# bayesian-object-tracking/dbot_ros

Hardware: AMD Instinct MI355X
Metric: particle-likelihoods/sec @640x480 (higher is better)
Workload: dtype f64; 1 GPU; C1: 2000 particles/GPU x loglikes(update=true), 640x480 synthetic depth frame, mesh m1 (5120 triangles), parents=permutation, 30-frame moving-object sequence, likelihood precision f64, window planes, inputs resident in HBM; particles_per_gpu=2000, triangles=5120

## Files before the change

dbot_ros_amd/csrc/rbsensor_capi.hip:

```cpp
#include "rbsensor_kernels.hip"
#include "rbsensor_tracker.hip"
#include "rbsensor_peers.hip"
#include "rbs_mesh.h"

#include "../../include/rbsensor_mi355x.h"

#include <dlfcn.h>
#include <unistd.h>
#if defined(__x86_64__)
#include <immintrin.h>
#endif

#include <cmath>
#include <cstdarg>
#include <cstddef>
#include <cstdio>
#include <cstdlib>
#include <cstring>
#include <algorithm>
#include <array>
#include <map>
#include <new>
#include <string>
#include <utility>
// ... 19 lines not shown
    double* d_soup = nullptr;
    float* d_frame = nullptr;
    double* d_aux = nullptr;
    double* d_aux_slot[2] = {nullptr, nullptr};
    float* d_pbg = nullptr;
    float* d_occ[2] = {nullptr, nullptr};
    int cur = 0;
    int pending_frames = 0;
    double* d_poses = nullptr;
    int* d_indices = nullptr;
    int* d_rects[2] = {nullptr, nullptr};
    rbs::Groups* d_groups[2] = {nullptr, nullptr};
    rbs::Strips* d_strips[2] = {nullptr, nullptr};
    int tracker_split_max = RBS_TRACKER_SPLIT_MAX_DEFAULT;
    bool copy_walk = false;
    int* d_parents[2] = {nullptr, nullptr};
    int4* d_win[2] = {nullptr, nullptr};
    int4* d_win_used = nullptr;
    int slab_px = 0;
    size_t plane_stride = 0;
    int4* d_reg[2] = {nullptr, nullptr};
    int* d_err = nullptr;
    int* h_err = nullptr;
    bool slab_auto = false;
    bool slab_probed = false;
    int* d_bbox = nullptr;
    bool windowed = true;
    bool many_clusters = false;
    unsigned char* d_wide_flags = nullptr;
    unsigned long long* d_area = nullptr;
    unsigned long long* h_area = nullptr;
    hipEvent_t ev_area = nullptr;
    bool area_pending = false;
    int area_n = 0;
    bool wide = false;
    double area_frac = 0.0;
    double mid_enter = 0.15;
    bool balance = true;
    int balance_blocks = 0;
    long balance_seen = 0;
    double wide_enter = 0.50, wide_leave = 0.35;
    int cu_count = 256;
    int smalln_target = 768;
    int rect_align = 4;
    int win_chunks = 8;
    int win_chunks_single = 2;
    int upload_chunks = 2;
    bool quiet = false;
    bool async_outstanding = false;
    float background = 0.f;
    int2* d_item_range = nullptr;
    int* d_item_particle = nullptr;
    int* d_ctr = nullptr;
    bool stp = false, stp_allowed = true;
    float* d_bgp[2] = {nullptr, nullptr};
    double stp_enter = 0.10;
    int stp_every = 32;
    long stp_last_rebase = -1000000;
    long stp_rebases = 0;
    long stp_block_until = 0;
    struct StpNow { int rebase = -1; bool entering = false; } stp_now;
    bool stp_leave_pending = false;
    int stp_request = -1;
    bool ipc_exported = false;
    int4* d_bgp_box = nullptr;
    bool split = false;
    unsigned* d_depth = nullptr;
    size_t depth_items = 0;
    int depth_blocks = 0, eval_blocks = 0;
    int* d_done = nullptr;
    double* d_partial = nullptr;
    unsigned long long* d_phase = nullptr;
    size_t partial_cap = 0;
    float* d_cluster_sphere = nullptr;
    float* d_cluster_cone = nullptr;
    double* d_cluster_vtx = nullptr;
    int* d_cluster_nv = nullptr;
    unsigned* d_tri_local = nullptr;
    float* d_vtx = nullptr;
    float* d_tri_plane = nullptr;
    int precision = RBS_PRECISION_F64;
    bool one_body_kernel = true;
    bool fused_copy = true;
    bool exact = false;
    int age_max = 0;
    double* d_ptab = nullptr;
    std::vector<double> ptab;
    long update_clock = 0;
    float* d_tmp_plane = nullptr;
    float* d_render = nullptr;
    unsigned char* h_in = nullptr;
    double* h_out = nullptr;
    unsigned char* d_in = nullptr;
    unsigned char* h_in_dev = nullptr;
    double* h_out_dev = nullptr;
    size_t in_idx_off = 0;
    hipEvent_t ev_out = nullptr;
    float* h_frames[2] = {nullptr, nullptr};
    float* h_frames_dev[2] = {nullptr, nullptr};
    size_t frame_pull_bytes = 128 * 1024;
    hipEvent_t ev_frame[2] = {nullptr, nullptr};
    hipStream_t up_stream = nullptr;
    float* d_fin[2] = {nullptr, nullptr};
    hipEvent_t ev_used[2] = {nullptr, nullptr};
    hipEvent_t ev_reader = nullptr;
    struct NextFrame {
        enum Kind { NONE, BORROWED_F64, BORROWED_F32, DEVICE, AHEAD } kind = NONE;
        const void* src = nullptr;
        hipStream_t stream = nullptr;
        int slot = -1;
        bool borrowed() const { return kind == BORROWED_F64 || kind == BORROWED_F32; }
    };
    struct FrameState {
        int cur = -1;
        int stage = 0;
        bool acquired = false;
        NextFrame next;
    } fr;
    hipStream_t stream = nullptr;
    hipStream_t copy_stream = nullptr;
    hipEvent_t ev_fork = nullptr;
    int copy_blocks = 1 << 30;
    int raster_blocks = 768;
    int copy_rows = 2;
    int copy_tpb = 64;
    const char* tile_override = nullptr;
    static constexpr int kRing = 256;
    hipEvent_t ev_start[kRing] = {}, ev_stop[kRing] = {}, ev_copy_start[kRing] = {}, ev_join[kRing] = {};
    hipEvent_t ev_raster_start[kRing] = {}, ev_raster_stop[kRing] = {}, ev_copy_stop[kRing] = {};
    bool ring_update[kRing] = {};
    int timing_every = 8;
    long timed_calls = 0;
    long calls = 0;
    int join_pending = -1;
    std::string err;
    bool poisoned = false;
    std::string poison_msg;
    int fault_shard = -1;
    long fault_call = -1, group_calls = 0;
    std::vector<rbs_handle*> shards;
    rbs_handle* group = nullptr;
    int shard_index = 0;
    int shard_cap = 0;
    hipEvent_t ev_done = nullptr;
    struct Rccl* rccl = nullptr;
    int peer_world = 0, peer_rank = 0;
    const float* peer_occ[rbs::kMaxDevices][2] = {};
    const int4* peer_win[rbs::kMaxDevices][2] = {};
    const int4* peer_reg[rbs::kMaxDevices][2] = {};
    void* peer_mapped[rbs::kMaxDevices][6] = {};
    void* d_peer_scratch = nullptr;
    size_t peer_scratch_bytes = 0;
    const float* snap_occ[rbs::kMaxDevices] = {};
    const int4* snap_win[rbs::kMaxDevices] = {};
    const int4* snap_reg[rbs::kMaxDevices] = {};
    rbs_config cfg{};
    std::vector<double> cfg_vertices;
    std::vector<int32_t> cfg_vertex_counts, cfg_triangles, cfg_triangle_counts;
    int occ_slots = 0;
};

struct Rccl {
    void* lib = nullptr;
    typedef void* comm_t;
    int (*CommInitAll)(comm_t*, int, const int*) = nullptr;
    int (*CommDestroy)(comm_t) = nullptr;
// ... 651 lines not shown
        const size_t bytes = sizeof(unsigned) * (size_t)rbs::kDepthTilePx * want;
        bool fits = bytes <= kDepthBudget;
        if (fits && want > h->depth_items) {
            size_t free_b = 0, total_b = 0;
            if (hipMemGetInfo(&free_b, &total_b) == hipSuccess) {
                const size_t mine = sizeof(unsigned) * (size_t)rbs::kDepthTilePx * h->depth_items;
                fits = bytes <= (free_b + mine) / 2;
            } else {
                (void)hipGetLastError();
            }
        }
        if (want > h->depth_items && fits) {
            RBS_HIP(h, hipStreamSynchronize(s));
            (void)hipFree(h->d_depth);
            h->d_depth = nullptr;
            h->depth_items = 0;
            if (hipMalloc(&h->d_depth, bytes) == hipSuccess) {
                h->depth_items = want;
            } else {
                (void)hipGetLastError();
                h->d_depth = nullptr;
                fits = false;
            }
        }
        if (want > h->depth_items && !fits) {
            split = false;
            if (have_borrowed) {
                if (int32_t rc = stage_borrowed(h)) return rc;
                P.frame = obs_frame(h);
                P.aux = obs_aux(h);
            }
        }
    }
    if (split) {
        P.depth = h->d_depth;
        P.depth_items = (int)std::min<size_t>(h->depth_items, 0x7fffffff);
        P.ctrb_this = h->d_ctr + 4 + (int)(h->calls & 1);
        P.ctrb_next = h->d_ctr + 4 + (int)((h->calls + 1) & 1);
    }
    int* const d_rects = h->d_rects[h->calls & 1];
    P.rects = d_rects;
    P.groups = h->d_groups[h->calls & 1];
    P.strips = update && h->windowed && !h->copy_walk ? h->d_strips[h->calls & 1] : nullptr;
    P.parents = h->d_parents[h->calls & 1];
    P.item_range = h->d_item_range;
    P.item_particle = h->d_item_particle;
    P.ctr_this = h->d_ctr + 2 * (int)(h->calls & 1);
    P.ctr_next = h->d_ctr + 2 * (int)((h->calls + 1) & 1);
    P.done = h->d_done;
    P.partial = h->d_partial;
#ifdef RBS_PHASE_TIMING
    if (!h->d_phase) { RBS_HIP(h, hipMalloc(&h->d_phase, 256)); RBS_HIP(h, hipMemset(h->d_phase, 0, 256)); }
    P.phase = h->d_phase;
#endif
    if (timed) RBS_HIP(h, hipEventRecord(h->ev_start[tslot], s));
    const dim3 block(rbs::kBlock);
    const dim3 pgrid((unsigned)((n + rbs::kPrepPerBlock - 1) / rbs::kPrepPerBlock));
    if (h->windowed && h->join_pending >= 0) {
        RBS_HIP(h, hipStreamWaitEvent(s, h->ev_join[h->join_pending], 0));
        h->join_pending = -1;
    }
    const float* rb_occ = P.occ_src; const int4* rb_win = P.win_src; const int4* rb_reg = h->slab_px ? P.reg_src : (const int4*)nullptr;
    int rb_local = rebase;
    if (rebase >= 0 && P.n_dev > 1) {
        const int owner = rebase / P.shard_cap;
        rb_local = rebase - owner * P.shard_cap;
        rb_occ = P.occ_src_dev[owner]; rb_win = P.win_src_dev[owner]; rb_reg = h->slab_px ? P.reg_src_dev[owner] : (const int4*)nullptr;
    }
    if (P.bgp_src) P.rebase_box = rebase >= 0 ? rb_win + rb_local : rebase == -2 ? h->d_bgp_box : nullptr;
    if (P.bgp_src && update)
        if (int32_t rc = launch_bgp_step(h, P, rb_occ, rb_win, rb_reg, rebase >= 0 ? rb_local : rebase, s)) return rc;
    bool sample_area = false;
    if (h->windowed && update) {
        sample_area = timed && !h->area_pending;
        if (sample_area) RBS_HIP(h, hipMemsetAsync(h->d_area, 0, sizeof(unsigned long long), s));
    }
    P.area_sum = sample_area ? h->d_area : nullptr;
    const bool wide = h->windowed && update && h->wide;
    const bool mid = h->windowed && update && !wide && h->area_frac > h->mid_enter;
    const bool fused = h->fused_copy && update && h->windowed && !wide && !mid && !split && !h->exact && !h->slab_px && !P.bgp_src &&
                       !P.groups && h->n_bodies == 1 && !h->many_clusters && !h->group && h->peer_world <= 1 && !h->ipc_exported &&
                       (h->precision == RBS_PRECISION_F32 || h->one_body_kernel);
    if (timed && fused) h->ring_update[tslot] = false;
    if (const float* df = take_device_frame(h, s)) {
        constexpr int ptb = 64 * rbs::kPrepPerBlock;
        const int aux_blocks = (h->d_aux || df != h->d_frame) ? (h->npx + ptb - 1) / ptb : 0;
        hipLaunchKernelGGL(rbs::rbs_frame_prep_kernel, dim3((unsigned)(aux_blocks + (n + rbs::kPrepPerBlock - 1) / rbs::kPrepPerBlock)), dim3(ptb), 0, s, P,
                           d_rects, update ? 1 : 0, df, h->d_aux, h->d_pbg, df == h->d_frame ? (float*)nullptr : h->d_frame, aux_blocks);
    } else {
        if (int32_t rc = flush_device_frame(h, s)) return rc;
        if (host_deltas) hipLaunchKernelGGL(rbs::rbs_prep_deltas_kernel, pgrid, dim3(64 * rbs::kPrepPerBlock), 0, s, P, d_rects, update ? 1 : 0);
        else hipLaunchKernelGGL(rbs::rbs_prep_kernel, pgrid, dim3(64 * rbs::kPrepPerBlock), 0, s, P, d_rects, update ? 1 : 0);
    }
    RBS_HIP(h, hipGetLastError());
    if (sample_area) {
        RBS_HIP(h, hipMemcpyAsync(h->h_area, h->d_area, sizeof(unsigned long long), hipMemcpyDeviceToHost, s));
        RBS_HIP(h, hipEventRecord(h->ev_area, s));
        h->area_pending = true;
        h->area_n = (n + 7) / 8;
    }
    if (update && !fused) {
        RBS_HIP(h, hipEventRecord(h->ev_fork, s));
        if (!(h->windowed && !wide)) RBS_HIP(h, hipStreamWaitEvent(h->copy_stream, h->ev_fork, 0));
    }
    if (h->join_pending >= 0) {
        RBS_HIP(h, hipStreamWaitEvent(s, h->ev_join[h->join_pending], 0));
        h->join_pending = -1;
    }
    if (h->balance && h->windowed && update && !wide && !mid && !fused && h->timed_calls > h->balance_seen && h->raster_blocks == 3 * h->cu_count) {
        const int last = (int)((h->timed_calls - 1) % rbs_handle::kRing);
        if (h->ring_update[last] && hipEventQuery(h->ev_raster_stop[last]) == hipSuccess && hipEventQuery(h->ev_copy_stop[last]) == hipSuccess) {
            float r_ms = 0.f, c_ms = 0.f;
            if (hipEventElapsedTime(&r_ms, h->ev_raster_start[last], h->ev_raster_stop[last]) == hipSuccess &&
                hipEventElapsedTime(&c_ms, h->ev_copy_start[last], h->ev_copy_stop[last]) == hipSuccess && r_ms > 0.f) {
                const int step = std::max(1, h->cu_count / 8), lo = 5 * h->cu_count / 2;
                int cur = h->balance_blocks ? h->balance_blocks : h->raster_blocks;
                if (c_ms > 1.04f * r_ms) cur = std::max(lo, cur - step);
                else if (c_ms < 0.92f * r_ms) cur = std::min(h->raster_blocks, cur + step);
                h->balance_blocks = cur;
            } else {
                (void)hipGetLastError();
            }
            h->balance_seen = h->timed_calls;
        }
    }
    const int full_grid = h->balance && h->balance_blocks && h->windowed && update && !fused ? h->balance_blocks : h->raster_blocks;
    const dim3 rgrid((unsigned)(wide || mid ? std::min(h->raster_blocks, 2 * h->cu_count) : full_grid));
    if (!split) if (int32_t rc = wait_for_upload(h, s)) return rc;
    bool window_copy_launched = false;
    auto launch_window_copy = [&]() -> int32_t {
        RBS_HIP(h, hipStreamWaitEvent(h->copy_stream, h->ev_fork, 0));
        if (timed) RBS_HIP(h, hipEventRecord(h->ev_copy_start[tslot], h->copy_stream));
        const int ny = std::min(n, 32768);
        const int strips = !RBS_COPY_STRIPS ? 0 : !P.groups ? 1 : (P.strips ? 2 : 0);
        const dim3 wg((unsigned)(strips == 1 ? h->win_chunks_single : h->win_chunks), (unsigned)ny, (unsigned)((n + ny - 1) / ny));
#define RBS_X3(S, B, E)                                                                                                             \
        do {                                                                                                                        \
            if (strips == 2) hipLaunchKernelGGL((rbs::rbs_copy_window_kernel<S, 2, B, E>), wg, dim3(64), 0, h->copy_stream, P);      \
            else if (strips == 1) hipLaunchKernelGGL((rbs::rbs_copy_window_kernel<S, 1, B, E>), wg, dim3(64), 0, h->copy_stream, P); \
            else hipLaunchKernelGGL((rbs::rbs_copy_window_kernel<S, 0, B, E>), wg, dim3(64), 0, h->copy_stream, P);                  \
        } while (0)
        switch ((h->exact ? 4 : 0) | (h->slab_px ? 2 : 0) | (P.bgp_src ? 1 : 0)) {
            case 0: RBS_X3(false, false, false); break;  case 1: RBS_X3(false, true, false); break;
            case 2: RBS_X3(true, false, false); break;   case 3: RBS_X3(true, true, false); break;
            case 4: RBS_X3(false, false, true); break;   case 5: RBS_X3(false, true, true); break;
            case 6: RBS_X3(true, false, true); break;    default: RBS_X3(true, true, true); break;
        }
#undef RBS_X3
        RBS_HIP(h, hipGetLastError());
        if (timed) RBS_HIP(h, hipEventRecord(h->ev_copy_stop[tslot], h->copy_stream));
        RBS_HIP(h, hipEventRecord(h->ev_join[slot], h->copy_stream));
        window_copy_launched = true;
        return RBS_OK;
    };
    if (timed) RBS_HIP(h, hipEventRecord(h->ev_raster_start[tslot], s));
    if (split) {
        const bool two = wide || mid;
        const dim3 dgrid((unsigned)(two ? std::min(h->depth_blocks, 2 * h->cu_count) : h->depth_blocks));
        const dim3 egrid((unsigned)(two ? std::min(h->eval_blocks, 3 * h->cu_count) : h->eval_blocks));
        const size_t dsm = rbs::smem_bytes_depth(P.tile_px, h->many_clusters), esm = rbs::smem_bytes(0, true, false, h->exact);
        if (h->many_clusters) hipLaunchKernelGGL((rbs::rbs_depth_kernel<true>), dgrid, block, dsm, s, P);
        else hipLaunchKernelGGL((rbs::rbs_depth_kernel<false>), dgrid, block, dsm, s, P);
        RBS_HIP(h, hipGetLastError());
        static const bool copy_first = [] { const char* e = std::getenv("RBS_SPLIT_COPY_FIRST"); return e ? std::atoi(e) != 0 : true; }();
        if (copy_first && have_borrowed && update && h->windowed && !wide)
            if (int32_t rc = launch_window_copy()) return rc;
// ... 461 lines not shown
    switch (cfg->likelihood_precision) {
        case RBS_PRECISION_DEFAULT:
            h->precision = RBS_PRECISION_LIBRARY_DEFAULT;
            if (const char* m = std::getenv("RBS_PRECISION")) {
                if (!std::strcmp(m, "f64")) h->precision = RBS_PRECISION_F64;
                else if (!std::strcmp(m, "f32")) h->precision = RBS_PRECISION_F32;
            }
            break;
        case RBS_PRECISION_F64: case RBS_PRECISION_F32: h->precision = cfg->likelihood_precision; break;
        default: return fail(h, RBS_ERR_INVALID_ARGUMENT, fmt("likelihood_precision %d", cfg->likelihood_precision));
    }
    if (cfg->state_layout < RBS_STATE_DEFAULT || cfg->state_layout > RBS_STATE_DENSE)
        return fail(h, RBS_ERR_INVALID_ARGUMENT, fmt("state_layout %d", cfg->state_layout));
    if (cfg->state_slab_px < RBS_SLAB_WHOLE_PLANES)
        return fail(h, RBS_ERR_INVALID_ARGUMENT, fmt("state_slab_px %d", cfg->state_slab_px));
    if (cfg->occlusion_mode < RBS_OCC_DEFAULT || cfg->occlusion_mode > RBS_OCC_REFERENCE)
        return fail(h, RBS_ERR_INVALID_ARGUMENT, fmt("occlusion_mode %d", cfg->occlusion_mode));

    DevParams& B = h->base;
    B.rows = h->rows; B.cols = h->cols; B.npx = h->npx;
    B.n_bodies = h->n_bodies;
    B.fx = K[0]; B.fy = K[4]; B.cx = K[2]; B.cy = K[5];
    B.tw = std::max(cfg->tail_weight, RBS_TAIL_WEIGHT_FLOOR); B.ms = cfg->model_sigma; B.sf = cfg->sigma_factor;
    B.lambda = -std::log(0.5) / rbs::kHalfLifeDepth;
    B.cv0 = (1.0 - B.tw) / std::sqrt(M_PI);
    B.bands = copy_bands_for(h->rows, h->cols);
    B.band_rows = (h->rows + B.bands - 1) / B.bands;

    rbs::PreparedMesh mesh;
    {
        const rbs::MeshInput in = {cfg->n_objects, cfg->vertices, cfg->vertex_counts, cfg->triangles, cfg->triangle_counts};
        const bool allow_cull = !(std::getenv("RBS_NO_CULL") && std::atoi(std::getenv("RBS_NO_CULL")));
        std::string why;
        if (const int rc = rbs::prepare_mesh(in, allow_cull, &mesh, &why)) return fail(h, rc, why);
        std::copy(std::begin(mesh.tri_begin), std::end(mesh.tri_begin), B.tri_begin);
        std::copy(std::begin(mesh.tri_end), std::end(mesh.tri_end), B.tri_end);
        std::copy(std::begin(mesh.vtx_begin), std::end(mesh.vtx_begin), B.vtx_begin);
        for (int b = 0; b < h->n_bodies; ++b) {
            B.body_cull[b] = mesh.body_cull[b];
            std::copy(mesh.sphere[b], mesh.sphere[b] + 4, B.sphere[b]);
        }
        B.n_tri = (int)mesh.n_alloc;
    }
    {
        size_t nv = 0, nt = 0;
        for (int b = 0; b < cfg->n_objects; ++b) { nv += (size_t)cfg->vertex_counts[b]; nt += (size_t)cfg->triangle_counts[b]; }
        h->cfg = *cfg;
        h->cfg_vertices.assign(cfg->vertices, cfg->vertices + 3 * nv);
        h->cfg_vertex_counts.assign(cfg->vertex_counts, cfg->vertex_counts + cfg->n_objects);
        h->cfg_triangles.assign(cfg->triangles, cfg->triangles + 3 * nt);
        h->cfg_triangle_counts.assign(cfg->triangle_counts, cfg->triangle_counts + cfg->n_objects);
        h->cfg.vertices = h->cfg_vertices.data();
        h->cfg.vertex_counts = h->cfg_vertex_counts.data();
        h->cfg.triangles = h->cfg_triangles.data();
        h->cfg.triangle_counts = h->cfg_triangle_counts.data();
        h->cfg.n_devices = 0;
        h->cfg.device_ids = nullptr;
    }
    h->many_clusters |= mesh.max_clusters > 64 * (rbs::kBlock / 64);
    if (const char* e = std::getenv("RBS_SHARED_CULL")) h->many_clusters = std::atoi(e) != 0;

    const size_t plane = (size_t)h->npx * sizeof(float);
    RBS_HIP(h, hipStreamCreateWithFlags(&h->stream, hipStreamNonBlocking));
    RBS_HIP(h, hipStreamCreateWithFlags(&h->copy_stream, hipStreamNonBlocking));
    RBS_HIP(h, hipEventCreateWithFlags(&h->ev_fork, hipEventDisableTiming));
    for (int i = 0; i < rbs_handle::kRing; ++i) {
        RBS_HIP(h, hipEventCreate(&h->ev_start[i]));
        RBS_HIP(h, hipEventCreate(&h->ev_stop[i]));
        RBS_HIP(h, hipEventCreate(&h->ev_copy_start[i]));
        RBS_HIP(h, hipEventCreate(&h->ev_join[i]));
        RBS_HIP(h, hipEventCreate(&h->ev_raster_start[i]));
        RBS_HIP(h, hipEventCreate(&h->ev_raster_stop[i]));
        RBS_HIP(h, hipEventCreate(&h->ev_copy_stop[i]));
    }
    {
        hipDeviceProp_t prop;
        RBS_HIP(h, hipGetDeviceProperties(&prop, h->device));
        h->cu_count = std::max(1, prop.multiProcessorCount);
        h->raster_blocks = 3 * h->cu_count;
        if (const char* m = std::getenv("RBS_RASTER_BLOCKS")) h->raster_blocks = std::max(1, std::atoi(m));
        if (const char* m = std::getenv("RBS_SHARED_TRAIL")) h->stp_allowed = std::atoi(m) != 0;
        if (const char* m = std::getenv("RBS_ONE_BODY")) h->one_body_kernel = std::atoi(m) != 0;
        if (const char* m = std::getenv("RBS_FUSED_COPY")) h->fused_copy = std::atoi(m) != 0;
        if (const char* m = std::getenv("RBS_TRACKER_SPLIT_MAX")) h->tracker_split_max = std::atoi(m);
        if (const char* m = std::getenv("RBS_STP_ENTER")) h->stp_enter = std::atof(m);
        if (const char* m = std::getenv("RBS_STP_EVERY")) h->stp_every = std::max(1, std::atoi(m));
        h->split = RBS_SPLIT_DEFAULT != 0;
        if (const char* m = std::getenv("RBS_SPLIT")) h->split = std::atoi(m) != 0;
        h->depth_blocks = RBS_DEPTH_MINWAVES * h->cu_count;
        h->eval_blocks = RBS_EVAL_MINWAVES * h->cu_count;
        if (const char* m = std::getenv("RBS_DEPTH_BLOCKS")) h->depth_blocks = std::max(1, std::atoi(m));
        if (const char* m = std::getenv("RBS_EVAL_BLOCKS")) h->eval_blocks = std::max(1, std::atoi(m));
        h->tile_override = std::getenv("RBS_TILE");
        if (const char* m = std::getenv("RBS_COPY_ROWS")) h->copy_rows = std::atoi(m);
        if (const char* m = std::getenv("RBS_COPY_TPB")) h->copy_tpb = std::max(64, std::atoi(m) / 64 * 64);
        if (cfg->state_layout == RBS_STATE_DENSE) h->windowed = false;
        else if (cfg->state_layout == RBS_STATE_DEFAULT)
            if (const char* m = std::getenv("RBS_STATE")) h->windowed = std::strcmp(m, "dense") != 0;
        h->smalln_target = 2 * std::max(1, prop.multiProcessorCount);
        if (const char* m = std::getenv("RBS_SMALLN_TARGET")) h->smalln_target = std::max(1, std::atoi(m));
        if (const char* m = std::getenv("RBS_MID_ENTER")) h->mid_enter = std::atof(m);
        if (const char* m = std::getenv("RBS_BALANCE")) h->balance = std::atoi(m) != 0;
        if (const char* m = std::getenv("RBS_WIDE_ENTER")) { h->wide_enter = std::atof(m); h->wide_leave = h->wide_enter * 0.67; }
        if (const char* m = std::getenv("RBS_RECT_ALIGN")) h->rect_align = std::atoi(m) >= 16 ? 16 : (std::atoi(m) >= 8 ? 8 : 4);
        if (const char* m = std::getenv("RBS_TIMING_EVERY")) h->timing_every = std::max(1, std::atoi(m));
        if (const char* m = std::getenv("RBS_WIN_CHUNKS")) h->win_chunks = h->win_chunks_single = std::min(1024, std::max(1, std::atoi(m)));
        if (const char* m = std::getenv("RBS_UPLOAD_CHUNKS")) h->upload_chunks = std::min(16, std::max(1, std::atoi(m)));
        if (h->cols & 3) h->windowed = false;
        h->base.rect_align = h->windowed ? h->rect_align : rbs::kRectAlign;
        if (!h->windowed && !std::getenv("RBS_RASTER_BLOCKS")) h->raster_blocks = 2 * std::max(1, prop.multiProcessorCount);
    }
    if (int32_t rc = upload(h, &h->d_soup, mesh.soup)) return rc;
    B.soup = h->d_soup;
    RBS_HIP(h, hipMalloc(&h->d_frame, plane));
    if (h->precision == RBS_PRECISION_F64) {
        RBS_HIP(h, hipMalloc(&h->d_aux, sizeof(double) * rbs::AUX_PLANES * (size_t)h->npx));
        RBS_HIP(h, hipMalloc(&h->d_aux_slot[0], sizeof(double) * rbs::AUX_PLANES * (size_t)h->npx));
        RBS_HIP(h, hipMalloc(&h->d_aux_slot[1], sizeof(double) * rbs::AUX_PLANES * (size_t)h->npx));
        RBS_HIP(h, hipMalloc(&h->d_pbg, plane));
    }
    RBS_HIP(h, hipMalloc(&h->d_render, plane));
    {
        int mode = cfg->occlusion_mode;
        const bool ages_fit = std::exp((65534.0 * h->delta_time) * std::log(h->p_oo - h->p_ov)) <= kExactTau;
        const bool can = h->precision == RBS_PRECISION_F64 && h->windowed && ages_fit;
        if (mode == RBS_OCC_REFERENCE && h->precision == RBS_PRECISION_F64 && h->windowed && !ages_fit)
            return fail(h, RBS_ERR_UNSUPPORTED, fmt("occlusion_mode REFERENCE keeps a 16-bit age per pixel: with p_occluded_occluded - p_occluded_visible = %.6g and "
                                                    "delta_time = %.6g a value has not decayed to 2^-40 of itself after 65 534 frames", h->p_oo - h->p_ov, h->delta_time));
        if (mode == RBS_OCC_DEFAULT) {
            mode = RBS_OCC_LIBRARY_DEFAULT;
            if (const char* m = std::getenv("RBS_OCC")) mode = !std::strcmp(m, "reference") ? RBS_OCC_REFERENCE : !std::strcmp(m, "device") ? RBS_OCC_DEVICE_RULE : mode;
            if (mode == RBS_OCC_REFERENCE && !can) mode = RBS_OCC_DEVICE_RULE;
        } else if (mode == RBS_OCC_REFERENCE && !can) {
            return fail(h, RBS_ERR_UNSUPPORTED, "occlusion_mode REFERENCE needs the binary64 likelihood (likelihood_precision F64) and the windowed "
                                                "state layout (cols a multiple of 4)");
        }
        h->exact = mode == RBS_OCC_REFERENCE;
    }
    if (h->exact) {
        const double cc = h->p_oo - h->p_ov, lc = std::log(cc);
        int K = 0;
        while (K < 65534 && std::exp(((double)K * h->delta_time) * lc) > kExactTau) ++K;
        h->age_max = K;
        h->ptab.resize(2 * (size_t)(K + 1));
        for (int a = 0; a <= K; ++a) {
            const double dt = (double)a * h->delta_time;
            const double pow_c = std::exp(dt * lc);
            h->ptab[2 * a] = pow_c;
            h->ptab[2 * a + 1] = (1.0 - h->p_oo) * (pow_c - 1.0) / (cc - 1.0);
        }
        RBS_HIP(h, hipMalloc(&h->d_ptab, sizeof(double) * h->ptab.size()));
        RBS_HIP(h, hipMemcpy(h->d_ptab, h->ptab.data(), sizeof(double) * h->ptab.size(), hipMemcpyHostToDevice));
        RBS_HIP(h, hipMalloc(&h->d_tmp_plane, plane));
    }
    h->slab_px = 0;
    if (h->windowed && cfg->state_slab_px > 0 && cfg->state_slab_px < h->npx)
        h->slab_px = std::max(1024, (cfg->state_slab_px + 3) & ~3);
    else if (h->windowed && cfg->state_slab_px == 0 && h->max_particles > 8192 && (h->cols & 3) == 0 && h->npx / 8 >= 4096) {
        h->slab_px = (h->npx / 8 + 3) & ~3;
        h->slab_auto = true;
    }
    if (h->slab_px >= h->npx) h->slab_px = 0;
    h->plane_stride = h->slab_px ? (size_t)h->slab_px : (size_t)h->npx;
    if (h->exact) h->plane_stride = exact_stride(h->plane_stride);
    const size_t occ_slots = h->occ_slots > 0 ? (size_t)h->occ_slots : (size_t)h->max_particles;
    RBS_HIP(h, hipMalloc(&h->d_occ[0], occ_alloc_bytes(sizeof(float) * h->plane_stride * occ_slots)));
// ... 2204 lines not shown
```

dbot_ros_amd/csrc/rbsensor_kernels.hip:

```cpp
#pragma once
#include <hip/hip_runtime.h>
#include <math.h>
#include <stdint.h>

#include "rbs_math.h"

namespace rbs {

#ifndef RBS_TILE_PX
#define RBS_TILE_PX 11008
#endif
#ifndef RBS_COPY_UNROLL
#define RBS_COPY_UNROLL 8
#endif
#ifndef RBS_NT
#define RBS_NT 1
#endif
#ifndef RBS_BIG_THRESH
#define RBS_BIG_THRESH 96
#endif
#ifndef RBS_EDGE_FILTER
#define RBS_EDGE_FILTER 0
#endif
#ifndef RBS_PIN_EDGES
#define RBS_PIN_EDGES 1
#endif
#ifndef RBS_SHARE_VERTICES
#define RBS_SHARE_VERTICES 1
#endif

#ifndef RBS_BLOCK
#define RBS_BLOCK 256
#endif
constexpr int kBlock = RBS_BLOCK;
constexpr int kTilePx = RBS_TILE_PX;
constexpr int kTilePxBig = 16384;
#ifndef RBS_MATH_LDS
#define RBS_MATH_LDS 1
#endif
constexpr int kMathTabDoubles = RBS_MATH_LDS ? rbsm::kErfcIntervals * rbsm::kErfcCoefs + rbsm::kLogIntervals * 2 : 0;
constexpr int kMathTabPx = (kMathTabDoubles * 8 + 63) / 64 * 16;
constexpr int kTilePxF64 = kTilePx - kMathTabPx, kTilePxBigF64 = kTilePxBig - kMathTabPx;
#ifndef RBS_BIG_CAP
#define RBS_BIG_CAP 256
#endif
constexpr int kBigCap = RBS_BIG_CAP;
constexpr int kBigThresh = RBS_BIG_THRESH;
constexpr int kCopyUnroll = RBS_COPY_UNROLL;
#ifndef RBS_SCAN_UNROLL
#define RBS_SCAN_UNROLL 2
#endif
#ifndef RBS_SCAN_UNROLL_F64
#define RBS_SCAN_UNROLL_F64 2
#endif
constexpr int kQPlanes_ = 4;
constexpr int kEvalQueue = 128;
constexpr int kTq = kQPlanes_ * kEvalQueue;
#ifndef RBS_RASTER_VGPRS
#define RBS_RASTER_VGPRS 80
#endif
#ifndef RBS_PRETEST_CLUSTERS
#define RBS_PRETEST_CLUSTERS 4
#endif
constexpr int kPre = RBS_PRETEST_CLUSTERS;
static_assert(kPre * 64 + 63 <= kTq && (kTq & (kTq - 1)) == 0, "the triangle ring must hold a step's survivors");
constexpr int kCullSteps = 28;
constexpr int kQPlanes = kQPlanes_;
constexpr int kRectAlign = 16;
constexpr float kSnapTau = 0x1p-18f;
typedef float floatx4 __attribute__((ext_vector_type(4)));
constexpr unsigned kInfBits = 0x7f800000u;
constexpr int kMaxBodies = 16;
constexpr int kMaxDevices = 8;
constexpr double kMaxDepth = 6.0;
constexpr double kHalfLifeDepth = 1.0;

constexpr int kMaxGroups = 4;
struct Groups {
    int n, pad0, pad1, pad2;
    int4 rect[kMaxGroups];
    int first[kMaxGroups];
    unsigned mask[kMaxGroups];
};

constexpr int kMaxStrips = (2 * kMaxGroups + 1) * (kMaxGroups + 1);
struct Strips {
    int n, pad0, pad1, pad2;
    int first[kMaxStrips + 1];
    ushort4 box[kMaxStrips];
};

struct DevParams {
    int rows, cols, npx;
    int n_bodies;
    int n_tri;
    int tri_begin[kMaxBodies + 1];
    int tri_end[kMaxBodies];
    const floatx4* tri_plane;
    const floatx4* vtx;
    int vtx_begin[kMaxBodies + 1];
    const float* cluster_sphere;
    const float* cluster_cone;
    const double* cluster_vtx;
    const int* cluster_nv;
    const unsigned* tri_local;
    int body_cull[kMaxBodies];
    int tile_px;
    int rect_align;
    int tile_w, tile_h;
    double fx, fy, cx, cy;
    double sphere[kMaxBodies][4];
    const double* soup;
    const float* frame;
    const double* aux;
    const float* pbg;
    double tw, ms, sf, lambda;
    double cv0;
    float alpha, beta;
    float bg_old, bg_new;
    int windowed;
    const int4* win_src;
    int4* win_dst;
    int4* win_used;
    unsigned long long* area_sum;
    unsigned char* wide_flags;
    int n_dev, shard_cap;
    const float* occ_src_dev[kMaxDevices];
    const int4* win_src_dev[kMaxDevices];
    const int4* reg_src_dev[kMaxDevices];
    int slab_px;
    int plane_stride;
    const int4* reg_src;
    int4* reg_dst;
    int* err;
    const float* occ_src;
    float* occ_dst;
    const double* poses;
    const double* poses_src;
    const double* deltas_src;
    const int* indices;
    int* parents;
    int slots;
    double* out;
    int n;
    int bands, band_rows;
    const int* rects;
    Groups* groups;
    Strips* strips;
    int2* item_range;
    int* item_particle;
    int* ctr_this;
    int* ctr_next;
    double* partial;
    int* done;
    const float* bgp_src;
    const float* bgp_dst;
    const int4* rebase_box;
    unsigned* depth;
    int depth_items;
    int* ctrb_this;
    int* ctrb_next;
    int exact;
    int plane_px;
    unsigned elapsed2;
    int age_max;
    const double* ptab;
#ifdef RBS_PHASE_TIMING
    unsigned long long* phase;
#endif
};
#ifdef RBS_PHASE_TIMING
__shared__ unsigned long long g_phase_lds[32];
#define RBS_TICK(k) do { if (threadIdx.x == 0) { const unsigned long long t_ = clock64(); g_phase_lds[k] += t_ - tick_; tick_ = t_; } } while (0)
#define RBS_COUNT(k, v) do { if (threadIdx.x == 0) g_phase_lds[k] += (unsigned long long)(v); } while (0)
#define RBS_TICK_DECL unsigned long long tick_ = clock64()
#define RBS_TICK_PARAM , unsigned long long& tick_
#define RBS_TICK_ARG , tick_
#else
#define RBS_TICK(k) do {} while (0)
#define RBS_COUNT(k, v) do {} while (0)
#define RBS_TICK_DECL do {} while (0)
#define RBS_TICK_PARAM
#define RBS_TICK_ARG
#endif

struct Rect { int x0, y0, x1, y1; };

struct TileGrid { int tw, th, nx, ny; };
__host__ __device__ inline TileGrid tile_grid(int rw, int rh, int max_w, int cap_px)
{
    TileGrid g;
    g.nx = (rw + max_w - 1) / max_w;
    if (g.nx < 1) g.nx = 1;
    g.tw = ((rw + g.nx - 1) / g.nx + 15) & ~15;
    if (g.tw < 16) g.tw = 16;
    int hmax = cap_px / g.tw;
    if (hmax < 1) hmax = 1;
    g.ny = (rh + hmax - 1) / hmax;
    if (g.ny < 1) g.ny = 1;
    g.th = (rh + g.ny - 1) / g.ny;
    if (g.th < 1) g.th = 1;
    return g;
}

__device__ inline float occ_step(float alpha, float beta, float v, float bg_new)
{
    const float x = fmaf(alpha, v, beta);
    return fabsf(x - bg_new) <= kSnapTau ? bg_new : x;
}

typedef unsigned short ushort2v __attribute__((ext_vector_type(2)));
constexpr unsigned kAgeBg2 = 0xffffffffu;
__device__ inline unsigned age_add2(unsigned packed, unsigned e2)
{
    return __builtin_bit_cast(unsigned, __builtin_elementwise_add_sat(__builtin_bit_cast(ushort2v, packed), __builtin_bit_cast(ushort2v, e2)));
}
__device__ inline float exact_prior(const DevParams& P, float v, int age)
{
    typedef double doublex2 __attribute__((ext_vector_type(2)));
    const doublex2 t = reinterpret_cast<const doublex2*>(P.ptab)[min(age, P.age_max)];
    const double new_visible = t.x * (1.0 - (double)v) + t.y;
    const float pr = (float)(1.0 - new_visible);
    return age > P.age_max ? P.bg_new : pr;
}
__device__ inline bool exact_differs(float v, unsigned a, float bv, unsigned ba, unsigned age_max)
{
    return a > age_max ? ba <= age_max : (a != ba || v != bv);
}

// ... 1180 lines not shown
                u = make_int4(P.cols, P.rows, 0, 0);
                seed = u;
                atomicExch(P.err, 1);
            }
            P.reg_dst[i] = u;
        }
        P.win_used[i] = u;
        P.win_dst[i] = seed;
        if (P.strips && P.groups) {
            Strips* S = P.strips + i;
            int* ys = ys_s[w];
            int ny = 0, ns = 0, total = 0;
            const int ng_ = G.n;
            if (u.z > u.x && u.w > u.y) {
                ys[ny++] = u.y;
                for (int g = 0; g < ng_; ++g) {
                    const int4 R = G.rect[g];
                    for (int e = 0; e < 2; ++e) {
                        const int y = min(max(e ? R.w : R.y, u.y), u.w);
                        int k = ny;
                        while (k > 0 && ys[k - 1] > y) --k;
                        if (k > 0 && ys[k - 1] == y) continue;
                        for (int m = ny; m > k; --m) ys[m] = ys[m - 1];
                        ys[k] = y; ++ny;
                    }
                }
                if (ys[ny - 1] != u.w) ys[ny++] = u.w;
                for (int bnd = 0; bnd + 1 < ny; ++bnd) {
                    const int ya = ys[bnd], yb = ys[bnd + 1];
                    int cur = u.x;
                    for (;;) {
                        int best = -1, bx = u.z;
                        for (int g = 0; g < ng_; ++g) {
                            const int4 R = G.rect[g];
                            if (R.z > R.x && R.y <= ya && R.w >= yb && R.z > cur && max(R.x, u.x) < bx) { best = g; bx = max(R.x, u.x); }
                        }
                        const int x1 = best < 0 ? u.z : bx;
                        if (x1 > cur) {
                            S->first[ns] = total;
                            S->box[ns] = make_ushort4((unsigned short)(cur >> 2), (unsigned short)(x1 >> 2), (unsigned short)ya, (unsigned short)yb);
                            total += ((x1 - cur) >> 2) * (yb - ya);
                            ++ns;
                        }
                        if (best < 0) break;
                        cur = max(cur, min(G.rect[best].z, u.z));
                        if (cur >= u.z) break;
                    }
                }
            }
            S->first[ns] = total;
            S->n = ns;
        }
        if (P.area_sum && (i & 7) == 0 && u.z > u.x && u.w > u.y)
            atomicAdd(P.area_sum, (unsigned long long)(u.z - u.x) * (unsigned long long)(u.w - u.y));
    }
}


__global__ __launch_bounds__(64 * kPrepPerBlock) void rbs_prep_kernel(const DevParams P, int* __restrict__ rects, int update)
{
    prep_particles(P, (int)blockIdx.x, rects, update);
}
__global__ __launch_bounds__(64 * kPrepPerBlock) void rbs_prep_deltas_kernel(const DevParams P, int* __restrict__ rects, int update)
{
    prep_particles<true>(P, (int)blockIdx.x, rects, update);
}

__global__ __launch_bounds__(64 * kPrepPerBlock) void rbs_frame_prep_kernel(const DevParams P, int* __restrict__ rects, int update,
                                      const float* __restrict__ frame_src, double* __restrict__ aux,
                                      float* __restrict__ pbg, float* __restrict__ keep, int aux_blocks)
{
    const int prep_blocks = (int)gridDim.x - aux_blocks;
    if ((int)blockIdx.x < prep_blocks) {
        prep_particles(P, (int)blockIdx.x, rects, update);
    } else {
        const int i = ((int)blockIdx.x - prep_blocks) * (int)blockDim.x + (int)threadIdx.x;
        if (i < P.npx) frame_aux_pixel(i, frame_src, aux, pbg, P.npx, P.tw, P.ms, P.sf, P.lambda, keep);
    }
}

#ifndef RBS_FCOPY_UNROLL
#define RBS_FCOPY_UNROLL 2
#endif
__device__ __forceinline__ void fused_window_copy(const DevParams& P, int particle)
{
    constexpr int kU = RBS_FCOPY_UNROLL;
    const int parent = P.parents[particle];
    if ((unsigned)parent >= (unsigned)P.slots) return;
    const int4 u = P.win_used[particle];
    if (u.z <= u.x || u.w <= u.y) return;
    const int4 q = reinterpret_cast<const int4*>(P.rects)[particle];
    const bool has = q.z > q.x;
    const int w4 = (u.z - u.x) >> 2, ux4 = u.x >> 2, W4 = P.cols >> 2;
    const int ty1 = has ? q.y : u.w, tby0 = has ? q.w : u.w;
    const int left4 = has ? (q.x - u.x) >> 2 : 0, right4 = has ? (u.z - q.z) >> 2 : 0, m = left4 + right4;
    const int rjump = has ? (q.z - u.x) >> 2 : 0;
    const int n_top = (ty1 - u.y) * w4, n_mid = (tby0 - ty1) * m, L = n_top + n_mid + (u.w - tby0) * w4;
    if (L == 0) return;
    const float rw4 = 1.0f / (float)w4, rm = 1.0f / (float)max(m, 1);
    const int4 pw = parent_window(P, parent);
    const floatx4* __restrict__ s4 = reinterpret_cast<const floatx4*>(parent_plane(P, parent));
    floatx4* __restrict__ d4 = reinterpret_cast<floatx4*>(P.occ_dst + (size_t)particle * P.plane_stride);
    const float alpha = P.alpha, beta = P.beta, bg_new = P.bg_new;
    int bx0 = P.cols, by0 = P.rows, bx1 = 0, by1 = 0;
    for (int base = 0; base < L; base += kBlock * kU) {
        floatx4 v[kU];
        int pk[kU];
#pragma unroll
        for (int k = 0; k < kU; ++k) {
            const int idx = base + k * kBlock + (int)threadIdx.x;
            const bool live = idx < L;
            const bool top = idx < n_top, mid = !top && idx < n_top + n_mid;
            const int j = top ? idx : mid ? idx - n_top : idx - n_top - n_mid, d = mid ? m : w4;
            int r = (int)((float)j * (mid ? rm : rw4));
            r += (r + 1) * d <= j ? 1 : 0;
            r -= r * d > j ? 1 : 0;
            const int kk = j - r * d;
            const int row = (top ? u.y : mid ? ty1 : tby0) + r, c4 = mid ? (kk < left4 ? kk : kk - left4 + rjump) : kk;
            const int col = (ux4 + c4) << 2;
            const bool stored = live && col >= pw.x && col < pw.z && row >= pw.y && row < pw.w;
            pk[k] = ((live ? (stored ? 2 : 1) : 0) << 28) | (row << 14) | (ux4 + c4);
            if (stored) v[k] = __builtin_nontemporal_load(&s4[row * W4 + (ux4 + c4)]);
        }
#pragma unroll
        for (int k = 0; k < kU; ++k) {
            const int st_ = pk[k] >> 28, row_ = (pk[k] >> 14) & 0x3fff, at_ = pk[k] & 0x3fff;
            if (!st_) continue;
            floatx4 w;
            if (st_ == 2) {
                w.x = occ_step(alpha, beta, v[k].x, bg_new);
                w.y = occ_step(alpha, beta, v[k].y, bg_new);
                w.z = occ_step(alpha, beta, v[k].z, bg_new);
                w.w = occ_step(alpha, beta, v[k].w, bg_new);
            } else {
                w.x = w.y = w.z = w.w = bg_new;
            }
            __builtin_nontemporal_store(w, &d4[row_ * W4 + at_]);
            if (w.x != bg_new || w.y != bg_new || w.z != bg_new || w.w != bg_new) {
                const int col = at_ << 2;
                bx0 = min(bx0, col); bx1 = max(bx1, col + 4);
                by0 = min(by0, row_); by1 = max(by1, row_ + 1);
            }
        }
    }
#pragma unroll
    for (int off = 32; off > 0; off >>= 1) {
        bx0 = min(bx0, __shfl_xor(bx0, off)); by0 = min(by0, __shfl_xor(by0, off));
        bx1 = max(bx1, __shfl_xor(bx1, off)); by1 = max(by1, __shfl_xor(by1, off));
    }
    if ((threadIdx.x & 63) == 0 && bx1 > bx0) {
        int* wd = reinterpret_cast<int*>(&P.win_dst[particle]);
        atomicMin(wd + 0, bx0); atomicMin(wd + 1, by0);
        atomicMax(wd + 2, bx1); atomicMax(wd + 3, by1);
    }
}

#ifndef RBS_RASTER_MINWAVES_F64
#define RBS_RASTER_MINWAVES_F64 3
#endif
#ifndef RBS_RASTER_MINWAVES
#define RBS_RASTER_MINWAVES 3
#endif
constexpr size_t smem_bytes(int tile_px, bool math_tables, bool many = false, bool exact = false);
template <bool UPDATE, int PREC, bool SLAB, bool MANY = false, bool STP = false, bool EXACT = false, bool ONE = false, bool FCOPY = false>
__device__ __forceinline__ void raster_kernel_body(const DevParams& P)
{
    static_assert(!FCOPY || (UPDATE && !SLAB && !MANY && !STP && !EXACT), "the fused copy serves windowed whole planes, scalar background");
    extern __shared__ __attribute__((aligned(16))) unsigned char smem[];
    Smem m = carve(smem, P.tile_px, PREC == 0 && RBS_MATH_LDS);
    if (EXACT) {
        m.ageq = reinterpret_cast<int*>(smem + smem_bytes(P.tile_px, PREC == 0 && RBS_MATH_LDS, MANY));
        m.agetab = reinterpret_cast<double*>(m.ageq + (kBlock / 64) * kEvalQueue);
        for (int i = threadIdx.x; i < 2 * min(kLdsAges, P.age_max + 1); i += kBlock) m.agetab[i] = P.ptab[i];
    }
    const int total = P.ctr_this[0];
    if (blockIdx.x == 0 && threadIdx.x == 0) { P.ctr_next[0] = 0; P.ctr_next[1] = 0; }
    if (PREC == 0 && RBS_MATH_LDS) {
        constexpr int ne = rbsm::kErfcIntervals * rbsm::kErfcCoefs, nl = rbsm::kLogIntervals * 2;
        for (int i = threadIdx.x; i < ne; i += kBlock) m.mtab[i] = rbsm::kErfcTab[i];
        for (int i = threadIdx.x; i < nl; i += kBlock) m.mtab[ne + i] = rbsm::kLogTab[i];
    }
#ifdef RBS_PHASE_TIMING
    const unsigned long long c0_ = clock64(), w0_ = wall_clock64();
    if (threadIdx.x < 32) g_phase_lds[threadIdx.x] = 0;
#endif
    RBS_TICK_DECL;
    const int grid = (int)gridDim.x;
    const int static_end = grid;
    int item = (int)blockIdx.x;
    for (;;) {
        if (item >= total) break;
        RBS_TICK(7);
        const int particle = __builtin_amdgcn_readfirstlane(P.item_particle[item]);
        const int4 q = reinterpret_cast<const int4*>(P.rects)[particle];
        const Rect r = {q.x, q.y, q.z, q.w};
        const int2 range = P.item_range[particle];
        const int first = range.x;
        double part = 0.0;
        const bool draw = item + grid >= static_end;
        int ticket = -1;
#ifdef RBS_PHASE_TIMING
        if (threadIdx.x == 0 && q.x + range.y == -12345) P.out[0] = 0.0;
        RBS_TICK(15);
#endif
        if (ONE || P.groups == nullptr) {
            if (r.x1 > r.x0) part = raster_eval_tile<UPDATE, PREC, SLAB, MANY, 0, STP, EXACT, ONE>(P, particle, r, item - first, m, 0xffffffffu, draw, ticket);
        } else {
            const Groups* G = P.groups + particle;
            const int k = item - first, ng = __builtin_amdgcn_readfirstlane(G->n);
            int g = 0;
            for (int c = 1; c < ng; ++c) g += (k >= __builtin_amdgcn_readfirstlane(G->first[c])) ? 1 : 0;
            if (ng > 0) {
                const int4 gq = G->rect[g];
                const Rect gr = {__builtin_amdgcn_readfirstlane(gq.x), __builtin_amdgcn_readfirstlane(gq.y),
                                 __builtin_amdgcn_readfirstlane(gq.z), __builtin_amdgcn_readfirstlane(gq.w)};
                part = raster_eval_tile<UPDATE, PREC, SLAB, MANY, 0, STP, EXACT>(P, particle, gr, k - __builtin_amdgcn_readfirstlane(G->first[g]), m,
                                                      (unsigned)__builtin_amdgcn_readfirstlane((int)G->mask[g]), draw, ticket);
            }
        }
        if (threadIdx.x == 0) {
            const int cnt = range.y;
            if (cnt == 1) {
                P.out[particle] = part;
            } else {
                unsigned long long* pp = reinterpret_cast<unsigned long long*>(P.partial);
                const unsigned long long old = atomicExch(pp + item, (unsigned long long)__double_as_longlong(part));
                const int bump = old == 0xfff8deadbeef0000ull ? 2 : 1;
                if (atomicAdd(&P.done[particle], bump) == cnt - 1) {
                    double sum = 0.0;
                    for (int k = 0; k < cnt; ++k) sum += __longlong_as_double((long long)atomicOr(pp + first + k, 0ull));
                    P.out[particle] = sum;
                }
            }
        }
        if (FCOPY && item == first) fused_window_copy(P, particle);
        if (draw) {
            if (threadIdx.x == 0) {
                if (ticket < 0) ticket = atomicAdd(&P.ctr_this[1], 1);
                *m.item = static_end + ticket;
            }
            __syncthreads();
            item = __builtin_amdgcn_readfirstlane(*m.item);
        } else {
            item += grid;
            __syncthreads();
        }
#ifdef RBS_PHASE_TIMING
        tick_ = clock64();
#endif
    }
#ifdef RBS_PHASE_TIMING
    if (threadIdx.x == 0) {
        for (int k = 0; k < 32; ++k)
            if (k != 5 && k != 6) atomicAdd(&P.phase[k], g_phase_lds[k]);
        atomicAdd(&P.phase[5], clock64() - c0_);
        atomicAdd(&P.phase[6], wall_clock64() - w0_);
    }
#endif
}

template <bool UPDATE, bool SLAB>
__global__ __launch_bounds__(kBlock, RBS_RASTER_MINWAVES) __attribute__((amdgpu_num_vgpr(RBS_RASTER_VGPRS)))
void rbs_raster_kernel_f32(const DevParams P)
{
    raster_kernel_body<UPDATE, 1, SLAB>(P);
}
#ifndef RBS_RASTER_VGPRS_F64
#define RBS_RASTER_VGPRS_F64 80
#endif
#if RBS_RASTER_VGPRS_F64
#define RBS_F64_BUDGET __attribute__((amdgpu_num_vgpr(RBS_RASTER_VGPRS_F64)))
#else
#define RBS_F64_BUDGET
#endif
template <bool UPDATE, bool SLAB>
__global__ __launch_bounds__(kBlock, RBS_RASTER_MINWAVES_F64) RBS_F64_BUDGET void rbs_raster_kernel_f64(const DevParams P)
{
    raster_kernel_body<UPDATE, 0, SLAB>(P);
}
template <bool UPDATE, bool SLAB>
__global__ __launch_bounds__(kBlock, RBS_RASTER_MINWAVES_F64) RBS_F64_BUDGET void rbs_raster_kernel_one_f64(const DevParams P)
{
    raster_kernel_body<UPDATE, 0, SLAB, false, false, false, true>(P);
}
__global__ __launch_bounds__(kBlock, RBS_RASTER_MINWAVES_F64) RBS_F64_BUDGET void rbs_raster_kernel_wcopy_one_f64(const DevParams P)
{
    raster_kernel_body<true, 0, false, false, false, false, true, true>(P);
}
__global__ __launch_bounds__(kBlock, RBS_RASTER_MINWAVES) __attribute__((amdgpu_num_vgpr(RBS_RASTER_VGPRS)))
void rbs_raster_kernel_wcopy_f32(const DevParams P)
{
    raster_kernel_body<true, 1, false, false, false, false, false, true>(P);
}
template <bool UPDATE, bool SLAB, bool MANY>
__global__ __launch_bounds__(kBlock, RBS_RASTER_MINWAVES_F64) RBS_F64_BUDGET void rbs_raster_kernel_stp_f64(const DevParams P)
{
    raster_kernel_body<UPDATE, 0, SLAB, MANY, true>(P);
}
template <bool UPDATE, bool SLAB, bool MANY>
__global__ __launch_bounds__(kBlock, RBS_RASTER_MINWAVES) __attribute__((amdgpu_num_vgpr(RBS_RASTER_VGPRS)))
void rbs_raster_kernel_stp_f32(const DevParams P)
{
    raster_kernel_body<UPDATE, 1, SLAB, MANY, true>(P);
}
template <bool UPDATE, bool SLAB, bool MANY, bool STP>
__global__ __launch_bounds__(kBlock, RBS_RASTER_MINWAVES_F64) RBS_F64_BUDGET void rbs_raster_kernel_exact_f64(const DevParams P)
{
    raster_kernel_body<UPDATE, 0, SLAB, MANY, STP, true>(P);
}
template <bool UPDATE, bool SLAB, bool STP>
__global__ __launch_bounds__(kBlock, RBS_RASTER_MINWAVES_F64) RBS_F64_BUDGET void rbs_raster_kernel_exact_one_f64(const DevParams P)
{
    raster_kernel_body<UPDATE, 0, SLAB, false, STP, true, true>(P);
}
template <bool UPDATE, bool SLAB>
__global__ __launch_bounds__(kBlock, RBS_RASTER_MINWAVES) __attribute__((amdgpu_num_vgpr(RBS_RASTER_VGPRS)))
void rbs_raster_kernel_many_f32(const DevParams P)
{
// ... 708 lines not shown
```

Measured before the change: 10.81 million particle-likelihoods/s.

## Front-load fused window copies for leading particles onto dedicated blocks

Before entering the raster/eval item loop, blocks with role 1 or 2 in each group of three copy the parent windows for a contiguous range of leading particles. Those particles then skip their per-item fused copy. The range is sized by configurable a,b counts, defaulting to 0,20 for f64. This moves copy work ahead of the evaluation so it overlaps with the other blocks that go straight to evaluation, and the lead copies use a higher unroll. The cost is that those blocks start evaluating later, which can change load balance in the dynamic work queue.

```diff
diff --git a/dbot_ros_amd/csrc/rbs_copy_lead.h b/dbot_ros_amd/csrc/rbs_copy_lead.h
--- /dev/null
+++ b/dbot_ros_amd/csrc/rbs_copy_lead.h
@@ -0,0 +1,49 @@
+#pragma once
+
+#if defined(__HIPCC__) || defined(__CUDACC__)
+#define RBS_LEAD_HD __host__ __device__
+#else
+#define RBS_LEAD_HD
+#endif
+
+namespace rbs {
+
+constexpr int kCopyLeadMax = 64;
+
+struct CopyLead { int a, b; };
+
+inline bool parse_copy_lead(const char* s, CopyLead* out)
+{
+    if (!s) return false;
+    int v[2] = {0, 0};
+    for (int k = 0; k < 2; ++k) {
+        if (*s < '0' || *s > '9') return false;
+        while (*s >= '0' && *s <= '9') { v[k] = v[k] * 10 + (*s - '0'); if (v[k] > kCopyLeadMax) return false; ++s; }
+        if (k == 0) { if (*s != ',') return false; ++s; }
+    }
+    if (*s) return false;
+    out->a = v[0]; out->b = v[1];
+    return true;
+}
+
+RBS_LEAD_HD inline int copy_lead_end(int grid, int a, int b, int n)
+{
+    if (grid < 3 || a < 0 || b < 0 || n <= 0) return 0;
+    const long long cap = (long long)(grid / 3) * (long long)(a + b);
+    return cap < (long long)n ? (int)cap : n;
+}
+
+RBS_LEAD_HD inline void copy_lead_range(int block, int grid, int a, int b, int lead_end, int* p0, int* p1)
+{
+    *p0 = *p1 = 0;
+    if (block < 0 || block >= grid || a < 0 || b < 0 || lead_end <= 0) return;
+    const int t = block / 3, role = block - 3 * t;
+    if (role == 0 || t >= grid / 3) return;
+    const long long first = (long long)t * (long long)(a + b) + (role == 2 ? a : 0);
+    const long long last = first + (role == 2 ? b : a);
+    const long long e = (long long)lead_end;
+    *p0 = (int)(first < e ? first : e);
+    *p1 = (int)(last < e ? last : e);
+}
+
+}
diff --git a/dbot_ros_amd/csrc/rbsensor_capi.hip b/dbot_ros_amd/csrc/rbsensor_capi.hip
--- a/dbot_ros_amd/csrc/rbsensor_capi.hip
+++ b/dbot_ros_amd/csrc/rbsensor_capi.hip
@@ -125,6 +125,7 @@
     int precision = RBS_PRECISION_F64;
     bool one_body_kernel = true;
     bool fused_copy = true;
+    rbs::CopyLead copy_lead_f64 = {0, 20}, copy_lead_f32 = {0, 0};
     bool exact = false;
     int age_max = 0;
     double* d_ptab = nullptr;
@@ -942,6 +943,12 @@
                        !P.groups && h->n_bodies == 1 && !h->many_clusters && !h->group && h->peer_world <= 1 && !h->ipc_exported &&
                        (h->precision == RBS_PRECISION_F32 || h->one_body_kernel);
     if (timed && fused) h->ring_update[tslot] = false;
+    P.lead_a = P.lead_b = P.lead_end = 0;
+    if (fused) {
+        const rbs::CopyLead cl = h->precision == RBS_PRECISION_F32 ? h->copy_lead_f32 : h->copy_lead_f64;
+        P.lead_a = cl.a; P.lead_b = cl.b;
+        P.lead_end = rbs::copy_lead_end(h->raster_blocks, cl.a, cl.b, n);
+    }
     if (const float* df = take_device_frame(h, s)) {
         constexpr int ptb = 64 * rbs::kPrepPerBlock;
         const int aux_blocks = (h->d_aux || df != h->d_frame) ? (h->npx + ptb - 1) / ptb : 0;
@@ -1569,6 +1576,11 @@
         if (const char* m = std::getenv("RBS_SHARED_TRAIL")) h->stp_allowed = std::atoi(m) != 0;
         if (const char* m = std::getenv("RBS_ONE_BODY")) h->one_body_kernel = std::atoi(m) != 0;
         if (const char* m = std::getenv("RBS_FUSED_COPY")) h->fused_copy = std::atoi(m) != 0;
+        if (const char* m = std::getenv("RBS_COPY_LEAD")) {
+            rbs::CopyLead cl;
+            if (!rbs::parse_copy_lead(m, &cl)) return fail(h, RBS_ERR_INVALID_ARGUMENT, fmt("RBS_COPY_LEAD: expected \"a,b\" with 0 <= a, b <= %d", rbs::kCopyLeadMax));
+            h->copy_lead_f64 = h->copy_lead_f32 = cl;
+        }
         if (const char* m = std::getenv("RBS_TRACKER_SPLIT_MAX")) h->tracker_split_max = std::atoi(m);
         if (const char* m = std::getenv("RBS_STP_ENTER")) h->stp_enter = std::atof(m);
         if (const char* m = std::getenv("RBS_STP_EVERY")) h->stp_every = std::max(1, std::atoi(m));
diff --git a/dbot_ros_amd/csrc/rbsensor_kernels.hip b/dbot_ros_amd/csrc/rbsensor_kernels.hip
--- a/dbot_ros_amd/csrc/rbsensor_kernels.hip
+++ b/dbot_ros_amd/csrc/rbsensor_kernels.hip
@@ -3,6 +3,7 @@
 #include <math.h>
 #include <stdint.h>
 
+#include "rbs_copy_lead.h"
 #include "rbs_math.h"
 
 namespace rbs {
@@ -145,6 +146,7 @@
     int n;
     int bands, band_rows;
     const int* rects;
+    int lead_a, lead_b, lead_end;
     Groups* groups;
     Strips* strips;
     int2* item_range;
@@ -1491,9 +1493,12 @@
 #ifndef RBS_FCOPY_UNROLL
 #define RBS_FCOPY_UNROLL 2
 #endif
-__device__ __forceinline__ void fused_window_copy(const DevParams& P, int particle)
-{
-    constexpr int kU = RBS_FCOPY_UNROLL;
+#ifndef RBS_FCOPY_LEAD_UNROLL
+#define RBS_FCOPY_LEAD_UNROLL 6
+#endif
+template <int kU>
+__device__ __forceinline__ void window_copy_unit(const DevParams& P, int particle)
+{
     const int parent = P.parents[particle];
     if ((unsigned)parent >= (unsigned)P.slots) return;
     const int4 u = P.win_used[particle];
@@ -1597,6 +1602,11 @@
     const int grid = (int)gridDim.x;
     const int static_end = grid;
     int item = (int)blockIdx.x;
+    if (FCOPY) {
+        int p0, p1;
+        copy_lead_range((int)blockIdx.x, grid, P.lead_a, P.lead_b, P.lead_end, &p0, &p1);
+        for (int p = p0; p < p1; ++p) window_copy_unit<RBS_FCOPY_LEAD_UNROLL>(P, p);
+    }
     for (;;) {
         if (item >= total) break;
         RBS_TICK(7);
@@ -1642,7 +1652,7 @@
                 }
             }
         }
-        if (FCOPY && item == first) fused_window_copy(P, particle);
+        if (FCOPY && item == first && particle >= P.lead_end) window_copy_unit<RBS_FCOPY_UNROLL>(P, particle);
         if (draw) {
             if (threadIdx.x == 0) {
                 if (ticket < 0) ticket = atomicAdd(&P.ctr_this[1], 1);
```

Measured after the change: 10.83 million particle-likelihoods/s, median of 6. Within noise of the previous version (+0.2%).
